# ArjunNarayanan/ProximalPolicyOptimization.jl

Hardware: AMD Instinct MI355X
Metric: env-steps/sec end-to-end PPO (rollout+GAE+update), 4096 envs, 1/2/4/8 MI355X (higher is better)
Workload: dtype f32; 1 GPU; 4096 parallel synthetic rand-poly-shaped envs per GPU (Q=8,H=32,A=128,F=72 int8), 2x256 MLP policy fp32, T=128 steps/iteration, 4 epochs, minibatch 4096/GPU, gamma=1.0 eps=0.05 entropy_w=0.01 Adam 1e-4; returns mode (lambda=1,V=0); envs_per_gpu=4096, T=128, epochs=4, minibatch_per_gpu=4096, parallelism=dp1, rollouts_streamed_to_disk=False

## Files before the change

### proximalpolicyoptimization.jl_amd/csrc/ppo_optim.hip

```cpp
#include "ppo_internal.h"
#include "ppo_device.h"
#include <algorithm>
#include <cstring>
#include <type_traits>

struct ParamLayout {
    int F, HID, NT, FP, NI, NL2;
    int64_t offW1, offb1, offW2, offW3, offb3, np;
};

static ParamLayout layout_of(const ppo_policy_s* p) {
    ParamLayout L;
    L.F = p->F; L.HID = p->HID; L.NT = p->HID / 32; L.FP = ((p->F + 31) / 32) * 32; L.NI = L.FP / 32; L.NL2 = p->L - 1;
    L.offW1 = 0; L.offb1 = (int64_t)p->HID * p->F; L.offW2 = L.offb1 + p->HID;
    L.offW3 = L.offW2 + (int64_t)L.NL2 * ((int64_t)p->HID * p->HID + p->HID);
    L.offb3 = L.offW3 + (int64_t)PPO_OUT * p->HID; L.np = L.offb3 + PPO_OUT;
    return L;
}

__device__ void loss_reduce_block(const double* __restrict__ terms, int64_t B, double inv_Bg, double entropy_weight,
                                  float* __restrict__ grad_tail);

struct PackPtrs {
    float* w1p; float* w2p; float* w2tp; float* b1p; float* b2p; float* w3p; float* b3;
    uint16_t* w1b; uint16_t* w2b; uint16_t* w2tb; uint16_t* w3c; uint16_t* w3tb;
    uint16_t* w2x; uint16_t* w1x; uint16_t* w2fx;
};

struct AdamFuse { float* params; float* m; float* v; double eta, beta1, beta2, eps, bp1, bp2; float* hist2; int on; };
__device__ __forceinline__ void pack_one(const ParamLayout& L, const PackPtrs& P, int64_t i, float x);
__device__ __forceinline__ void adam_one(const AdamFuse& A, const ParamLayout& L, const PackPtrs& P, int64_t i, float g);

struct ChainFuse {
    float* params; float* hist2; int on; int n;
    int kind[4];
    double c[4][6];
    float* s0[4]; float* s1[4];
};
__device__ __forceinline__ void chain_one(const ChainFuse& C, const ParamLayout& L, const PackPtrs& P, int64_t i, float g);
__device__ __forceinline__ void fuse_one(const AdamFuse& A, const ParamLayout& L, const PackPtrs& P, int64_t i, float g) { adam_one(A, L, P, i, g); }
__device__ __forceinline__ void fuse_one(const ChainFuse& C, const ParamLayout& L, const PackPtrs& P, int64_t i, float g) { chain_one(C, L, P, i, g); }

struct ClipFuse {
    float* hist2; int on;
    ChainFuse C;
    float* dbuf;
    double* part;
};
__device__ __forceinline__ float chain_delta(const ChainFuse& C, int64_t i, float g);
__device__ __forceinline__ void clip_partial(double* __restrict__ part, size_t e, float d);

__device__ __forceinline__ void fuse_one(const ClipFuse&, const ParamLayout&, const PackPtrs&, int64_t, float) {}

template <typename Fuse>
__global__ __launch_bounds__(256) void k_grad_reduce(const float* __restrict__ slabs, size_t slab_stride, int nwg_w, int nwg_s, ParamLayout L,
                                                     float* __restrict__ grad, const double* __restrict__ terms, int64_t B,
                                                     double inv_Bg, double entropy_weight, Fuse A, PackPtrs P) {
    if (blockIdx.x == gridDim.x - 1) {
        loss_reduce_block(terms, B, inv_Bg, entropy_weight, grad + L.np);
        if (A.on && A.hist2 && threadIdx.x == 0) { A.hist2[0] = grad[L.np]; A.hist2[1] = grad[L.np + 1]; }
        return;
    }
    __shared__ float part[4][64];
    const int el = threadIdx.x & 63, grp = threadIdx.x >> 6;
    const size_t e = (size_t)blockIdx.x * 64 + el;
    const size_t nW2l = (size_t)L.HID * L.HID, nW2 = (size_t)L.NL2 * nW2l, nW1 = (size_t)L.HID * L.FP;
    const size_t total = nW2 + nW1 + (size_t)L.HID * (1 + L.NL2) + (size_t)L.HID * 4 + 4;
    float ps[8] = {0.f, 0.f, 0.f, 0.f, 0.f, 0.f, 0.f, 0.f};
    const int nwg = (e < nW2 + nW1) ? nwg_w : nwg_s;
    bool dead = false;
    if (e >= nW2 && e < nW2 + nW1) {
        const size_t e1 = e - nW2;
        const int it = (int)((e1 >> 10) % L.NI);
        dead = 32 * it + (int)(e1 & 31) >= L.F;
    }
    if (e < total && !dead) {
        int g = grp;
        for (; g + 28 < nwg; g += 32) {
#pragma unroll
            for (int u = 0; u < 8; ++u) ps[u] += slabs[(size_t)(g + 4 * u) * slab_stride + e];
        }
        for (int u = 0; g < nwg; g += 4, ++u) ps[u] += slabs[(size_t)g * slab_stride + e];
    }
    part[grp][el] = ((ps[0] + ps[1]) + (ps[2] + ps[3])) + ((ps[4] + ps[5]) + (ps[6] + ps[7]));
    __syncthreads();
    constexpr bool clip = std::is_same<Fuse, ClipFuse>::value;
    if (grp != 0 || (e >= total && !clip)) return;
    const float s = (part[0][el] + part[1][el]) + (part[2][el] + part[3][el]);
    int64_t canon = -1;
    if (e < nW2) {
        const int lay = (int)(e / nW2l);
        const size_t el2 = e - (size_t)lay * nW2l;
        const int lane = (int)(el2 & 63), r = (int)((el2 >> 6) & 15);
        const int tile = (int)(el2 >> 10), kt = tile % L.NT, ft = tile / L.NT;
        const int f = dfeat(ft, r, lane >> 5), k = 32 * kt + (lane & 31);
        canon = L.offW2 + (int64_t)lay * ((int64_t)nW2l + L.HID) + f + (int64_t)L.HID * k;
    } else if (e < nW2 + nW1) {
        const size_t e1 = e - nW2;
        const int lane = (int)(e1 & 63), r = (int)((e1 >> 6) & 15);
        const int tile = (int)(e1 >> 10), it = tile % L.NI, ft = tile / L.NI;
        const int ko = dfeat(ft, r, lane >> 5), i = 32 * it + (lane & 31);
        if (i < L.F) canon = L.offW1 + ko + (int64_t)L.HID * i;
    } else {
        size_t e2 = e - nW2 - nW1;
        if (e2 < (size_t)L.HID) canon = L.offb1 + (int64_t)e2;
        else if ((e2 -= L.HID) < (size_t)L.HID * L.NL2)
            canon = L.offW2 + (int64_t)(e2 / L.HID) * ((int64_t)nW2l + L.HID) + (int64_t)nW2l + (int64_t)(e2 % L.HID);
        else if ((e2 -= (size_t)L.HID * L.NL2) < (size_t)L.HID * 4) canon = L.offW3 + (int64_t)(e2 & 3) + 4 * (int64_t)(e2 >> 2);
        else canon = L.offb3 + (int64_t)(e2 - (size_t)L.HID * 4);
    }
    if constexpr (clip) {
        float d = 0.f;
        if (e < total && canon >= 0) {
            grad[canon] = s;
            d = chain_delta(A.C, canon, s);
            A.dbuf[canon] = d;
        }
        clip_partial(A.part, e, d);
        return;
    }
    if (canon >= 0) {
        grad[canon] = s;
        if (A.on) fuse_one(A, L, P, canon, s);
    }
}

__device__ void loss_reduce_block(const double* __restrict__ terms, int64_t B, double inv_Bg, double entropy_weight,
                                  float* __restrict__ grad_tail) {
    __shared__ double s0[256], s1[256];
    const double2* t2 = reinterpret_cast<const double2*>(terms);
    double a[8] = {0, 0, 0, 0, 0, 0, 0, 0}, b[8] = {0, 0, 0, 0, 0, 0, 0, 0};
    int64_t i = threadIdx.x;
    for (; i + 7 * 256 < B; i += 8 * 256) {
#pragma unroll
        for (int u = 0; u < 8; ++u) { const double2 v = t2[i + u * 256]; a[u] += v.x; b[u] += v.y; }
    }
    for (int u = 0; i < B; i += 256, ++u) { const double2 v = t2[i]; a[u] += v.x; b[u] += v.y; }
    s0[threadIdx.x] = ((a[0] + a[1]) + (a[2] + a[3])) + ((a[4] + a[5]) + (a[6] + a[7]));
    s1[threadIdx.x] = ((b[0] + b[1]) + (b[2] + b[3])) + ((b[4] + b[5]) + (b[6] + b[7]));
    __syncthreads();
    for (int off = 128; off >= 1; off >>= 1) {
        if ((int)threadIdx.x < off) { s0[threadIdx.x] += s0[threadIdx.x + off]; s1[threadIdx.x] += s1[threadIdx.x + off]; }
        __syncthreads();
    }
    if (threadIdx.x == 0) {
        grad_tail[0] = (float)(-(s0[0] * inv_Bg));
        grad_tail[1] = (float)(entropy_weight * (-(s1[0] * inv_Bg)));
    }
}


__device__ __forceinline__ uint16_t to_bf16(float x) { return __builtin_bit_cast(uint16_t, (__bf16)x); }
__device__ __forceinline__ void split3_bf16(float x, uint16_t& ph, uint16_t& pm, uint16_t& pl) {
    ph = to_bf16(x);
    const float r1 = x - __uint_as_float((uint32_t)ph << 16);
    pm = to_bf16(r1);
    const float r2 = r1 - __uint_as_float((uint32_t)pm << 16);
    pl = to_bf16(r2);
}
__device__ __forceinline__ void acc_kslot(int kk, int& s, int& hh, int& jj) {
    const int q = kk & 15;
    s = kk >> 4; hh = (q >> 2) & 1; jj = 4 * (q >> 3) + (q & 3);
}

__device__ __forceinline__ void pack_one(const ParamLayout& L, const PackPtrs& P, int64_t i, float x) {
    const int HID = L.HID, F = L.F, NT = L.NT;
    if (i < L.offb1) {
        const int io = (int)(i % HID), k = (int)(i / HID);
        const int hh = k / (F / 2), s = k % (F / 2);
        P.w1p[((size_t)((io >> 5) * (F / 8) + (s >> 2)) * 64 + (io & 31) + 32 * hh) * 4 + (s & 3)] = x;
        if (P.w1x) {
            uint16_t ph, pm, pl;
            split3_bf16(x, ph, pm, pl);
            uint16_t* base = P.w1x + ((size_t)(io >> 5) * 5 + (k >> 4)) * 3 * 512 + ((size_t)(io & 31) + 32 * ((k >> 3) & 1)) * 8 + (k & 7);
            base[0] = pl; base[512] = pm; base[1024] = ph;
        }
        if (P.w1b) {
            const int KS1 = (F + 15) / 16;
            P.w1b[((size_t)((io >> 5) * KS1 + (k >> 4)) * 64 + (io & 31) + 32 * ((k >> 3) & 1)) * 8 + (k & 7)] = to_bf16(x);
        }
    } else if (i < L.offW2) {
        const int f = (int)(i - L.offb1), kk = f & 31, hh = (kk >> 2) & 1, r = (kk & 3) + 4 * (kk >> 3);
        P.b1p[((f >> 5) * 2 + hh) * 16 + r] = x;
    } else if (i < L.offW3) {
        const int64_t per = (int64_t)HID * HID + HID;
        const int lay = (int)((i - L.offW2) / per);
        const int64_t e = (i - L.offW2) - (int64_t)lay * per;
        if (e >= (int64_t)HID * HID) {
            const int f = (int)(e - (int64_t)HID * HID), kk = f & 31, hh = (kk >> 2) & 1, r = (kk & 3) + 4 * (kk >> 3);
            P.b2p[(size_t)lay * HID + ((f >> 5) * 2 + hh) * 16 + r] = x;
            return;
        }
        const size_t lo = (size_t)lay * HID * HID;
        const int f = (int)(e % HID), k = (int)(e / HID);
        {
            const int kk = k & 31, hh = (kk >> 2) & 1, r = (kk & 3) + 4 * (kk >> 3);
            const int s = 16 * (k >> 5) + r;
            P.w2p[lo + ((size_t)((f >> 5) * (HID / 8) + (s >> 2)) * 64 + (f & 31) + 32 * hh) * 4 + (s & 3)] = x;
        }
        {
            const bool zrow = PPO_BWD_Z2ROW_AT(HID);
            const int g = f >> 3, hh = zrow ? (f >> 2) & 1 : f & 1, e = zrow ? f & 3 : (f >> 1) & 3;
            P.w2tp[lo + ((size_t)((k >> 5) * (HID / 8) + g) * 64 + (k & 31) + 32 * hh) * 4 + e] = x;
        }
        if (P.w2x && lay == 0) {
            uint16_t ph, pm, pl;
            split3_bf16(x, ph, pm, pl);
            const int KS = HID / 16;
            int s, hh, jj;
            {
                acc_kslot(f & 31, s, hh, jj);
                uint16_t* base = P.w2x + ((size_t)(k >> 5) * KS + 2 * (f >> 5) + s) * 3 * 512 + ((size_t)(k & 31) + 32 * hh) * 8 + jj;
                base[0] = pl; base[512] = pm; base[1024] = ph;
            }
            {
                acc_kslot(k & 31, s, hh, jj);
                uint16_t* base = P.w2fx + ((size_t)(f >> 5) * KS + 2 * (k >> 5) + s) * 3 * 512 + ((size_t)(f & 31) + 32 * hh) * 8 + jj;
                base[0] = pl; base[512] = pm; base[1024] = ph;
            }
        }
        if (P.w2b) {
            const uint16_t xb = to_bf16(x);
            int s, hh, jj;
            acc_kslot(k & 31, s, hh, jj);
            P.w2b[((size_t)((f >> 5) * (HID / 16) + 2 * (k >> 5) + s) * 64 + (f & 31) + 32 * hh) * 8 + jj] = xb;
            P.w2tb[((size_t)((k >> 5) * (HID / 16) + (f >> 4)) * 64 + (k & 31) + 32 * ((f >> 3) & 1)) * 8 + (f & 7)] = xb;
        }
    } else if (i < L.offb3) {
        const int64_t e = i - L.offW3;
        const int oo = (int)(e & 3), k = (int)(e >> 2);
        const int kk = k & 31, hh = (kk >> 2) & 1, r = (kk & 3) + 4 * (kk >> 3);
        P.w3p[((size_t)(hh * NT + (k >> 5)) * 16 + r) * 4 + oo] = x;
        if (P.w3c) {
            const uint16_t xb = to_bf16(x);
            int s, h2, jj;
            acc_kslot(k & 31, s, h2, jj);
            P.w3c[((size_t)((2 * (k >> 5) + s) * 2 + h2) * 4 + oo) * 8 + jj] = xb;
            P.w3tb[(size_t)k * 4 + oo] = xb;
        }
    } else {
        P.b3[i - L.offb3] = x;
    }
}

__device__ __forceinline__ void adam_one(const AdamFuse& A, const ParamLayout& L, const PackPtrs& P, int64_t i, float g) {
    const double gd = (double)g;
    const float mn = (float)(A.beta1 * (double)A.m[i] + (1.0 - A.beta1) * gd);
    const float vn = (float)(A.beta2 * (double)A.v[i] + ((1.0 - A.beta2) * gd) * gd);
    A.m[i] = mn; A.v[i] = vn;
    const double delta = (double)mn / (1.0 - A.bp1) / (sqrt((double)vn / (1.0 - A.bp2)) + A.eps) * A.eta;
    const float x = A.params[i] - (float)delta;
    A.params[i] = x;
    pack_one(L, P, i, x);
}

__global__ void k_pack_params(const float* __restrict__ params, ParamLayout L, PackPtrs P) {
    const int64_t i = (int64_t)blockIdx.x * blockDim.x + threadIdx.x;
    if (i >= L.np) return;
    pack_one(L, P, i, params[i]);
}

__global__ void k_adam(float* __restrict__ params, const float* __restrict__ grad, float* __restrict__ m,
                       float* __restrict__ v, ParamLayout L, PackPtrs P, double eta, double beta1, double beta2,
                       double eps, double bp1, double bp2, float* __restrict__ hist2) {
    const int64_t i = (int64_t)blockIdx.x * blockDim.x + threadIdx.x;
    if (hist2 && i < 2) hist2[i] = grad[L.np + i];
    if (i >= L.np) return;
    const double gd = (double)grad[i];
    const float mn = (float)(beta1 * (double)m[i] + (1.0 - beta1) * gd);
    const float vn = (float)(beta2 * (double)v[i] + ((1.0 - beta2) * gd) * gd);
    m[i] = mn; v[i] = vn;
    const double delta = (double)mn / (1.0 - bp1) / (sqrt((double)vn / (1.0 - bp2)) + eps) * eta;
    const float x = params[i] - (float)delta;
    params[i] = x;
    pack_one(L, P, i, x);
}

__device__ __forceinline__ float chain_delta(const ChainFuse& C, int64_t i, float g) {
    float d = g;
#pragma unroll
    for (int j = 0; j < 4; ++j) {
        if (j >= C.n) break;
        const double* c = C.c[j];
        const double dd = (double)d;
        const int kind = C.kind[j];
        if (kind == PPO_OPT_ADAM) {
            float* m = C.s0[j];
            float* v = C.s1[j];
            const float mn = (float)(c[1] * (double)m[i] + (1.0 - c[1]) * dd);
            const float vn = (float)(c[2] * (double)v[i] + ((1.0 - c[2]) * dd) * dd);
            m[i] = mn; v[i] = vn;
            d = (float)((double)mn / (1.0 - c[4]) / (sqrt((double)vn / (1.0 - c[5])) + c[3]) * c[0]);
        } else if (kind == PPO_OPT_EXPDECAY || kind == PPO_OPT_DESCENT) {
            d = (float)(dd * c[0]);
        } else if (kind == PPO_OPT_MOMENTUM) {
            const float vn = (float)(c[1] * (double)C.s0[j][i] - c[0] * dd);
            C.s0[j][i] = vn;
            d = -vn;
        } else if (kind == PPO_OPT_NESTEROV) {
            const double v0 = (double)C.s0[j][i];
            const double dn = (c[1] * c[1]) * v0 - ((1.0 + c[1]) * c[0]) * dd;
            C.s0[j][i] = (float)(c[1] * v0 - c[0] * dd);
            d = (float)(-dn);
        } else if (kind == PPO_OPT_RMSPROP) {
            const float a = (float)(c[1] * (double)C.s0[j][i] + ((1.0 - c[1]) * dd) * dd);
            C.s0[j][i] = a;
            const float ra = (float)sqrt((double)a);
            d = (float)(dd * (c[0] / ((double)ra + c[2])));
        } else if (kind == PPO_OPT_CLIPVALUE) {
            d = (float)(dd > c[0] ? c[0] : (dd < -c[0] ? -c[0] : dd));
        } else if (kind == PPO_OPT_WEIGHTDECAY) {
            d = (float)(dd + c[0] * (double)C.params[i]);
        } else {
            d = (float)(dd * c[0]);
        }
    }
    return d;
}

__device__ __forceinline__ void dd_add(double& h, double& l, double bh, double bl) {
    const double s = h + bh;
    if (!isfinite(s)) { h = s; l = 0.0; return; }
    const double v = s - h;
    double e = (h - (s - v)) + (bh - v);
    e += l + bl;
    h = s + e;
    l = e - (h - s);
}

__device__ __forceinline__ void clip_partial(double* __restrict__ part, size_t e, float d) {
    double h = (double)d * (double)d, l = 0.0;
#pragma unroll
    for (int off = 16; off >= 1; off >>= 1) {
        const double bh = __shfl_down(h, off, 32), bl = __shfl_down(l, off, 32);
        dd_add(h, l, bh, bl);
    }
    if ((e & 31) == 0) { part[2 * (e >> 5)] = h; part[2 * (e >> 5) + 1] = l; }
}

__device__ __forceinline__ void chain_one(const ChainFuse& C, const ParamLayout& L, const PackPtrs& P, int64_t i, float g) {
    const float x = C.params[i] - chain_delta(C, i, g);
    C.params[i] = x;
    pack_one(L, P, i, x);
}

__global__ void k_chain_update(const float* __restrict__ grad, ParamLayout L, PackPtrs P, ChainFuse C) {
    const int64_t i = (int64_t)blockIdx.x * blockDim.x + threadIdx.x;
    if (C.hist2 && i < 2) C.hist2[i] = grad[L.np + i];
    if (i >= L.np) return;
    chain_one(C, L, P, i, grad[i]);
}

__global__ __launch_bounds__(256) void k_chain_clip1(const float* __restrict__ grad, ParamLayout L, ClipFuse A) {
    const int64_t i = (int64_t)blockIdx.x * blockDim.x + threadIdx.x;
    if (A.hist2 && i < 2) A.hist2[i] = grad[L.np + i];
    float d = 0.f;
    if (i < L.np) {
        d = chain_delta(A.C, i, grad[i]);
        A.dbuf[i] = d;
    }
    clip_partial(A.part, (size_t)i, d);
}

#define PPO_CLIP_MAX_ARRAYS 10
struct ClipMap {
    const float* dbuf; const double* part;
    double thresh;
    int na;
    int64_t start[PPO_CLIP_MAX_ARRAYS + 1];
    int32_t s0[PPO_CLIP_MAX_ARRAYS], s1[PPO_CLIP_MAX_ARRAYS];
};
__device__ __forceinline__ int clip_array(const ClipMap& M, int64_t i) {
    int a = 0;
    while (a + 1 < M.na && i >= M.start[a + 1]) ++a;
    return a;
}

#define PPO_CLIP_BLOCK 256
__global__ __launch_bounds__(PPO_CLIP_BLOCK) void k_clip_apply(ParamLayout L, PackPtrs P, ChainFuse C, ClipMap M) {
    __shared__ double wsum[PPO_CLIP_BLOCK / 64][2];
    __shared__ float nrm[PPO_CLIP_MAX_ARRAYS];
    const int t = threadIdx.x, lane = t & 63, w = t >> 6;
    const int64_t i0 = (int64_t)blockIdx.x * PPO_CLIP_BLOCK, i = i0 + t;
    const int a0 = clip_array(M, i0), a1 = clip_array(M, std::min<int64_t>(i0 + PPO_CLIP_BLOCK, L.np) - 1);
// ... 279 lines not shown
```

### proximalpolicyoptimization.jl_amd/csrc/ppo_policy_bwd_x6.hip

```cpp
#include "ppo_internal.h"
#include "ppo_device.h"
#include <cstdlib>

#include "ppo_x6.h"
typedef float pk2 __attribute__((ext_vector_type(2)));
__device__ __forceinline__ pk2 pk_fma(pk2 a, pk2 b, pk2 c) { return __builtin_elementwise_fma(a, b, c); }

struct BwdXArgs {
    unsigned long long* stamps;
    const int8_t* states; const int32_t* idx; int64_t B;
    int tps; int x_by_tile;
    const float4* act1; const float4* act2; const float4* dY;
    const uint4* w2x; const float4* w3p;
    float* slabs; size_t slab_stride;
};

template <int F, int HID>
struct XCfg {
    static_assert(F == 72, "state rows of 72 features (+ the ones column, zero padded to 96)");
    static constexpr int NT = HID / 32, KS = HID / 16;
    static constexpr int LD = 36;
    static constexpr int WG_PER_CU = HID == 128 ? 2 : 1;
    static constexpr int XROW = 80;
    static constexpr int NIX = 3;
    static constexpr size_t oZ2 = 0, szZ2 = (size_t)NT * 6 * 1024;
    static constexpr size_t oH2 = oZ2 + szZ2, szH2 = sizeof(float) * HID * LD;
    static constexpr size_t oH1 = oH2 + szH2, szH1 = (size_t)3 * NT * 2048;
    static constexpr size_t oX = oH1 + szH1, szX = (size_t)32 * NIX * XROW;
    static constexpr size_t oDY = oX + szX, oW3 = oDY + 512, oID = oW3 + (size_t)HID * 16, total = oID + 2048;
    static_assert(total <= 160 * 1024 / WG_PER_CU, "LDS budget");
};

#define X6_LANE() unsigned ln = (unsigned)lane; asm volatile("" : "+v"(ln)); const int j = (int)(ln & 31u), h = (int)(ln >> 5); (void)j; (void)h

#ifndef PPO_X6_DMA_SPREAD
#define PPO_X6_DMA_SPREAD 0
#endif
#ifndef PPO_X6_RING
#define PPO_X6_RING 6
#endif
#ifndef PPO_X6_RING_256
#define PPO_X6_RING_256 4
#endif

template <int F, int HID>
__global__ __launch_bounds__(HID * 2, 2) void k_policy_bwd_x6(BwdXArgs a) {
    using C = XCfg<F, HID>;
    constexpr int NT = C::NT, KS = C::KS, NTHR = NT * 64, LD = C::LD, NIX = C::NIX, XROW = C::XROW;
    constexpr int XQW = 32 * F / 8, XPD = (XQW + NTHR - 1) / NTHR;
    constexpr int RD = HID >= 256 ? PPO_X6_RING_256 : PPO_X6_RING;
    static_assert(NTHR >= 256 && NTHR >= HID, "shape");
    extern __shared__ __attribute__((aligned(16))) char smem_c[];
    char* const fragZ2 = smem_c + C::oZ2;
    float* const sH2 = reinterpret_cast<float*>(smem_c + C::oH2);
    char* const imgH1 = smem_c + C::oH1;
    char* const imgX = smem_c + C::oX;
    float* const sDY = reinterpret_cast<float*>(smem_c + C::oDY);
    float* const sW3 = reinterpret_cast<float*>(smem_c + C::oW3);
    uint4* const sID = reinterpret_cast<uint4*>(smem_c + C::oID);

    const int tid = threadIdx.x, lane = tid & 63;
    const int w = __builtin_amdgcn_readfirstlane(tid >> 6);
    const int j = lane & 31, h = lane >> 5;

    f32x16 accW2[NT], accW1[NIX];
#pragma unroll
    for (int kt = 0; kt < NT; ++kt)
#pragma unroll
        for (int r = 0; r < 16; ++r) accW2[kt][r] = 0.0f;
#pragma unroll
    for (int it = 0; it < NIX; ++it)
#pragma unroll
        for (int r = 0; r < 16; ++r) accW1[it][r] = 0.0f;
    float db2 = 0.f, db3 = 0.f, dw3[4] = {0.f, 0.f, 0.f, 0.f};

#ifdef PPO_X6_ZERO_LDS
    for (int i = tid; i < (int)(C::total / 4); i += NTHR) reinterpret_cast<uint32_t*>(smem_c)[i] = 0u;
    __syncthreads();
#endif
    if (tid < HID) {
        const int kk = tid & 31, hh = (kk >> 2) & 1, r = (kk & 3) + 4 * (kk >> 3);
        *reinterpret_cast<float4*>(&sW3[tid * 4]) = a.w3p[(size_t)(hh * NT + (tid >> 5)) * 16 + r];
    }
    if (tid < 64) {
        const int n = tid & 31, hB = tid >> 5, e = 4 * ((n >> 3) & 1) + (n & 3);
#pragma unroll
        for (int s1 = 0; s1 < 2; ++s1) {
            uint4 v = make_uint4(0u, 0u, 0u, 0u);
            if (hB == ((n >> 2) & 1) && s1 == (n >> 4)) {
                const uint32_t one = (e & 1) ? 0x3F800000u : 0x00003F80u;
                if ((e >> 1) == 0) v.x = one; else if ((e >> 1) == 1) v.y = one; else if ((e >> 1) == 2) v.z = one; else v.w = one;
            }
            sID[s1 * 64 + tid] = v;
        }
    }
    for (int i = tid; i < 32 * NIX * XROW / 4; i += NTHR) {
        const int row = i / (XROW / 4), c = i % (XROW / 4);
        reinterpret_cast<uint32_t*>(imgX)[i] = (row == F && c < 16) ? 0x3F803F80u : 0u;
    }
    __syncthreads();

    const char* const wx = reinterpret_cast<const char*>(a.w2x + (size_t)w * 3 * KS * 64);
    float* const h2slice = sH2 + (size_t)(32 * w) * LD;
    char* const z2own = fragZ2 + (size_t)w * 6 * 1024;
    const unsigned h2slice_lds = __builtin_amdgcn_readfirstlane((unsigned)(size_t)(__attribute__((address_space(3))) void*)h2slice);
    const unsigned z2own_lds = __builtin_amdgcn_readfirstlane((unsigned)(size_t)(__attribute__((address_space(3))) void*)z2own);
    auto dma_frag = [&](const float4* base, int64_t t, unsigned dst_lds, unsigned ln) {
        const float4* const sb = base + ((size_t)t * NT + w) * 4 * 64;
        const unsigned voff = ln * 16u;
#pragma unroll
        for (int q = 0; q < 4; ++q) {
            unsigned keep;
            const float4* gsrc = sb + q * 64;
            const unsigned dst = dst_lds + (unsigned)q * 1024u;
            asm volatile("s_mov_b32 %0, m0\n\ts_mov_b32 m0, %2\n\ts_nop 0\n\tglobal_load_lds_dwordx4 %1, %3 nt\n\ts_mov_b32 m0, %0"
                         : "=&s"(keep) : "v"(voff), "s"(dst), "s"(gsrc) : "memory");
        }
    };
    auto dma_one = [&](const float4* base, int64_t t, unsigned dst_lds, int q, unsigned ln) {
        unsigned keep;
        const float4* gsrc = base + ((size_t)t * NT + w) * 4 * 64 + ln + q * 64;
        const unsigned dst = dst_lds + (unsigned)q * 1024u;
        asm volatile("s_mov_b32 %0, m0\n\ts_mov_b32 m0, %2\n\ts_nop 0\n\tglobal_load_lds_dwordx4 %1, off nt\n\ts_mov_b32 m0, %0"
                     : "=&s"(keep) : "v"(gsrc), "s"(dst) : "memory");
    };
    (void)dma_one;
    float4 dy;
    uint2 xd[XPD];
    auto issue_tile_loads = [&](int64_t t, int sidx, unsigned ln) {
        dy = *reinterpret_cast<const float4*>(reinterpret_cast<const char*>(a.dY + (size_t)t * 32) + (ln & 31u) * 16u);
        const char* xs = reinterpret_cast<const char*>(a.states + (a.x_by_tile ? (size_t)t : ((size_t)sidx * a.tps + (size_t)(t % a.tps))) * 32 * F);
#pragma unroll
        for (int i = 0; i < XPD; ++i) {
            const unsigned u = (unsigned)(64 * w) + ln + (unsigned)i * NTHR;
            const unsigned d = (u & 31u) * (unsigned)(F / 8) + (u >> 5);
            xd[i] = u < (unsigned)XQW ? *reinterpret_cast<const uint2*>(xs + d * 8u) : make_uint2(0u, 0u);
        }
    };
    if ((int64_t)blockIdx.x < a.B) {
        dma_frag(a.act2, blockIdx.x, h2slice_lds, (unsigned)lane);
        dma_frag(a.act1, blockIdx.x, z2own_lds, (unsigned)lane);
        issue_tile_loads(blockIdx.x, a.x_by_tile ? 0 : __builtin_amdgcn_readfirstlane(a.idx[blockIdx.x / a.tps]), (unsigned)lane);
    }
    asm volatile("s_waitcnt vmcnt(0)" ::: "memory");
    __syncthreads();

#ifdef PPO_X6_STAMP
    unsigned long long st_sum[12] = {0, 0, 0, 0, 0, 0, 0, 0, 0, 0, 0, 0}, st_t = clock64();
#define XSTAMP(i) do { unsigned long long _n = clock64(); st_sum[i] += _n - st_t; st_t = _n; } while (0)
#else
#define XSTAMP(i) do {} while (0)
#endif
    for (int64_t tile = blockIdx.x; tile < a.B; tile += gridDim.x) {
        {
            X6_LANE();
            const unsigned hw = (unsigned)(w * 2048 + 64 * j), cx = (unsigned)(j >> 2) & 7u;
            float4 v1[4];
#pragma unroll
            for (int q = 0; q < 4; ++q) v1[q] = *reinterpret_cast<const float4*>(z2own + q * 1024 + ln * 16);
            asm volatile("s_waitcnt lgkmcnt(0)" ::: "memory");
#pragma unroll
            for (int q = 0; q < 4; ++q) {
                const float hv[4] = {v1[q].x, v1[q].y, v1[q].z, v1[q].w};
                uint2 ph, pm, pl;
                x_split4(hv, ph, pm, pl);
                const unsigned off = hw + 8u * (((unsigned)(2 * q + h)) ^ cx);
                *reinterpret_cast<uint2*>(imgH1 + off) = ph;
                *reinterpret_cast<uint2*>(imgH1 + NT * 2048 + off) = pm;
                *reinterpret_cast<uint2*>(imgH1 + 2 * NT * 2048 + off) = pl;
            }
        }
        __builtin_amdgcn_sched_barrier(0);
        XSTAMP(0);
        {
            X6_LANE();
            float* const h2b = sH2 + (32 * w + 4 * h) * LD + j;
            const float w3a0 = sW3[(32 * w + j) * 4 + h], w3a1 = sW3[(32 * w + j) * 4 + 2 + h];
            float4 v2[4];
#pragma unroll
            for (int q = 0; q < 4; ++q) v2[q] = *reinterpret_cast<const float4*>(h2slice + q * 256 + ln * 4);
            if (w == 0 && h == 0) *reinterpret_cast<float4*>(&sDY[j * 4]) = dy;
            f32x16 dh2;
#pragma unroll
            for (int r = 0; r < 16; ++r) dh2[r] = 0.0f;
            dh2 = __builtin_amdgcn_mfma_f32_32x32x2f32(w3a0, h ? dy.y : dy.x, dh2, 0, 0, 0);
            dh2 = __builtin_amdgcn_mfma_f32_32x32x2f32(w3a1, h ? dy.w : dy.z, dh2, 0, 0, 0);
            asm volatile("s_waitcnt lgkmcnt(0)" ::: "memory");
#pragma unroll
            for (int s = 0; s < 2; ++s) {
                uint2 zh[2], zm[2], zl[2];
#pragma unroll
                for (int qq = 0; qq < 2; ++qq) {
                    const int q = 2 * s + qq;
                    const float h2v[4] = {v2[q].x, v2[q].y, v2[q].z, v2[q].w};
                    float z[4];
#pragma unroll
                    for (int e = 0; e < 4; ++e) {
                        z[e] = dh2[4 * q + e] * (h2v[e] > 0.0f ? 1.0f : 0.01f);
                        h2b[(e + 8 * q) * LD] = h2v[e];
                    }
                    x_split4(z, zh[qq], zm[qq], zl[qq]);
                }
                *reinterpret_cast<uint4*>(z2own + (s * 3 + 0) * 1024 + ln * 16) = make_uint4(zh[0].x, zh[0].y, zh[1].x, zh[1].y);
                *reinterpret_cast<uint4*>(z2own + (s * 3 + 1) * 1024 + ln * 16) = make_uint4(zm[0].x, zm[0].y, zm[1].x, zm[1].y);
                *reinterpret_cast<uint4*>(z2own + (s * 3 + 2) * 1024 + ln * 16) = make_uint4(zl[0].x, zl[0].y, zl[1].x, zl[1].y);
                __builtin_amdgcn_sched_barrier(0);
            }
        }
        XSTAMP(1);
        {
        X6_LANE();
#pragma unroll
        for (int i = 0; i < XPD; ++i) {
            const int d = 64 * w + (int)ln + i * NTHR;
            if (d < XQW) {
                const int row = d & 31, c = d >> 5;
                const int slot = (row & 19) | ((row & 4) << 1) | ((row & 8) >> 1);
                const uint32_t xw[2] = {xd[i].x, xd[i].y};
                char* const xp = imgX + (8 * c) * XROW + 2 * slot;
#pragma unroll
                for (int e = 0; e < 8; ++e) {
                    const float xv = (float)(int)(int8_t)(xw[e >> 2] >> (8 * (e & 3)));
                    *reinterpret_cast<uint16_t*>(xp + e * XROW) = (uint16_t)(__float_as_uint(xv) >> 16);
                }
            }
        }
        }
        XSTAMP(2);
        __syncthreads();
        XSTAMP(3);
        auto small_grads = [&]() {
            X6_LANE();
            const float* gh = sH2 + (32 * w + j) * LD + 16 * h;
            const float* gy = sDY + 64 * h;
            pk2 d01 = {0.f, 0.f}, d23 = {0.f, 0.f};
#pragma unroll 1
            for (int rc = 0; rc < 16; rc += 4) {
                const float4 h4 = *reinterpret_cast<const float4*>(gh + rc);
                const float hv[4] = {h4.x, h4.y, h4.z, h4.w};
                float4 y[4];
#pragma unroll
                for (int i = 0; i < 4; ++i) y[i] = *reinterpret_cast<const float4*>(gy + (rc + i) * 4);
                __builtin_amdgcn_sched_barrier(0);
#pragma unroll
                for (int i = 0; i < 4; ++i) {
                    const pk2 hh2 = {hv[i], hv[i]};
                    d01 = pk_fma(pk2{y[i].x, y[i].y}, hh2, d01); d23 = pk_fma(pk2{y[i].z, y[i].w}, hh2, d23);
                }
                __builtin_amdgcn_sched_barrier(0);
            }
            dw3[0] += d01.x; dw3[1] += d01.y; dw3[2] += d23.x; dw3[3] += d23.y;
            if (w == 0 && ln < 4u) {
                float s = 0.f;
                for (int r = 0; r < 32; ++r) s += sDY[r * 4 + ln];
                db3 += s;
            }
        };
        uint4 ring[RD];
#pragma unroll
        for (int g = 0; g < RD; ++g) { unsigned lo = (unsigned)lane * 16u; asm volatile("" : "+v"(lo)); ring[g] = *reinterpret_cast<const uint4*>(wx + (lo + (unsigned)g * 1024u)); }
        const bool grads_first = (2 * w < NT);
        const int64_t ntile = (tile + gridDim.x < a.B) ? tile + gridDim.x : tile;
        if (grads_first) small_grads();
        XSTAMP(4);
        {
            f32x16 acc;
#pragma unroll
            for (int r = 0; r < 16; ++r) acc[r] = 0.0f;
            f32x16 accs;
#pragma unroll
            for (int r = 0; r < 16; ++r) accs[r] = 0.0f;
            unsigned wo = (unsigned)RD * 1024u;
            asm volatile("" : "+s"(wo));
            constexpr int RU = (RD % 3 == 0) ? RD / 3 : RD;
            static_assert(KS % RU == 0 && (3 * RU) % RD == 0, "ring rounds");
            static_assert(RD * 1024 <= PPO_X6_W2_PAD_BYTES, "the last ring round reads RD pieces past the end of the W2 stream");
            unsigned zo = (unsigned)lane * 16u;
            asm volatile("" : "+v"(zo));
            const char* zp = fragZ2 + zo;
            const unsigned lo16 = zo;
#pragma unroll 1
            for (int k0 = 0; k0 < KS; k0 += RU) {
#pragma unroll
                for (int u = 0; u < RU; ++u) {
                    const int s0 = (3 * u + 0) % RD, s1 = (3 * u + 1) % RD, s2 = (3 * u + 2) % RD;
                    const uint4 z_h = *reinterpret_cast<const uint4*>(zp + (u * 3 + 0) * 1024);
                    const uint4 z_m = *reinterpret_cast<const uint4*>(zp + (u * 3 + 1) * 1024);
                    const uint4 z_l = *reinterpret_cast<const uint4*>(zp + (u * 3 + 2) * 1024);
                    accs = x_mfma(z_h, ring[s0], accs);
                    __builtin_amdgcn_sched_barrier(0);
                    ring[s0] = *reinterpret_cast<const uint4*>(wx + (lo16 + wo));
                    __builtin_amdgcn_sched_barrier(0);
                    accs = x_mfma(z_m, ring[s1], accs);
                    accs = x_mfma(z_h, ring[s1], accs);
                    __builtin_amdgcn_sched_barrier(0);
                    ring[s1] = *reinterpret_cast<const uint4*>(wx + (lo16 + wo + 1024u));
                    __builtin_amdgcn_sched_barrier(0);
                    accs = x_mfma(z_l, ring[s2], accs);
                    accs = x_mfma(z_m, ring[s2], accs);
                    acc = x_mfma(z_h, ring[s2], acc);
                    __builtin_amdgcn_sched_barrier(0);
                    ring[s2] = *reinterpret_cast<const uint4*>(wx + (lo16 + wo + 2048u));
                    wo += 3 * 1024;
                    asm volatile("" : "+s"(wo));
                    __builtin_amdgcn_sched_barrier(0);
                }
                zp += RU * 3 * 1024;
            }
#pragma unroll
            for (int r = 0; r < 16; ++r) acc[r] = acc[r] + accs[r];
            XSTAMP(5);
            X6_LANE();
            const unsigned q4 = (ln & 15u) >> 2, p4 = ln & 3u, g1 = (ln >> 4) & 1u;
            typedef __attribute__((address_space(3))) xs16x4 lds_s16x4;
            uint2 zh[4], zm[4], zl[4];
#pragma unroll
            for (int g = 0; g < 4; ++g) {
                const unsigned r0 = 8u * g + 4u * h;
                const char* hp = imgH1 + w * 2048 + 64u * (r0 + q4) + 8u * ((4u * g1 + p4) ^ ((r0 >> 2) & 7u));
                const uint2 sg = __builtin_bit_cast(uint2, __builtin_amdgcn_ds_read_tr16_b64_v4i16((lds_s16x4*)(hp)));
                const float z1[4] = {acc[4 * g + 0] * ((int16_t)(sg.x & 0xFFFFu) > 0 ? 1.0f : 0.01f),
                                     acc[4 * g + 1] * ((int32_t)sg.x >= 0x10000 ? 1.0f : 0.01f),
                                     acc[4 * g + 2] * ((int16_t)(sg.y & 0xFFFFu) > 0 ? 1.0f : 0.01f),
                                     acc[4 * g + 3] * ((int32_t)sg.y >= 0x10000 ? 1.0f : 0.01f)};
                x_split4(z1, zh[g], zm[g], zl[g]);
            }
            const char* const xb = imgX + j * XROW + 16 * h;
#pragma unroll
            for (int s = 0; s < 2; ++s) {
                uint4 bx[NIX];
#pragma unroll
                for (int it = 0; it < NIX; ++it) bx[it] = *reinterpret_cast<const uint4*>(xb + 32 * it * XROW + 32 * s);
                const uint4 a_l = make_uint4(zl[2 * s].x, zl[2 * s].y, zl[2 * s + 1].x, zl[2 * s + 1].y);
                const uint4 a_m = make_uint4(zm[2 * s].x, zm[2 * s].y, zm[2 * s + 1].x, zm[2 * s + 1].y);
                const uint4 a_h = make_uint4(zh[2 * s].x, zh[2 * s].y, zh[2 * s + 1].x, zh[2 * s + 1].y);
#pragma unroll
                for (int it = 0; it < NIX; ++it) {
                    accW1[it] = x_mfma(a_l, bx[it], accW1[it]);
                    accW1[it] = x_mfma(a_m, bx[it], accW1[it]);
                    accW1[it] = x_mfma(a_h, bx[it], accW1[it]);
                }
            }
        }
        XSTAMP(6);
        if (!grads_first) small_grads();
        XSTAMP(7);
        __syncthreads();
        XSTAMP(8);
        {
            X6_LANE();
            uint4 ah[2], am[2], al[2];
            {
                const uint4 id0 = sID[ln], id1 = sID[64 + ln];
                float s2 = 0.f;
#pragma unroll
                for (int p = 2; p >= 0; --p) {
                    const uint4 f0 = *reinterpret_cast<const uint4*>(z2own + (0 * 3 + p) * 1024 + ln * 16);
                    const uint4 f1 = *reinterpret_cast<const uint4*>(z2own + (1 * 3 + p) * 1024 + ln * 16);
                    f32x16 t;
#pragma unroll
                    for (int r = 0; r < 16; ++r) t[r] = 0.0f;
                    t = x_mfma(f0, id0, t);
                    t = x_mfma(f1, id1, t);
                    float sp = 0.f;
#pragma unroll
                    for (int r = 0; r < 16; ++r) sp += t[r];
                    s2 += sp;
                    uint4 pk[2];
#pragma unroll
                    for (int s = 0; s < 2; ++s)
                        pk[s] = make_uint4(x_perm(t[8 * s + 0], t[8 * s + 1]), x_perm(t[8 * s + 2], t[8 * s + 3]),
                                           x_perm(t[8 * s + 4], t[8 * s + 5]), x_perm(t[8 * s + 6], t[8 * s + 7]));
                    if (p == 0) { ah[0] = pk[0]; ah[1] = pk[1]; } else if (p == 1) { am[0] = pk[0]; am[1] = pk[1]; } else { al[0] = pk[0]; al[1] = pk[1]; }
                }
                db2 += s2;
            }
            asm volatile("s_waitcnt lgkmcnt(0)" ::: "memory");
#if !(PPO_X6_DMA_SPREAD & 1)
            dma_frag(a.act2, ntile, h2slice_lds, ln);
#endif
#if !(PPO_X6_DMA_SPREAD & 2)
            dma_frag(a.act1, ntile, z2own_lds, ln);
#endif
            {
                int nidx = 0;
                if (!a.x_by_tile) {
                    const int32_t* ip = a.idx + ntile / a.tps;
                    asm volatile("s_load_dword %0, %1, 0x0\n\ts_waitcnt lgkmcnt(0)" : "=s"(nidx) : "s"(ip) : "memory");
                }
                issue_tile_loads(ntile, nidx, ln);
            }
            unsigned tb[2][2];
            {
                const unsigned q4 = (ln & 15u) >> 2, p4 = ln & 3u, g1 = (ln >> 4) & 1u;
#pragma unroll
                for (int s = 0; s < 2; ++s)
#pragma unroll
                    for (int u = 0; u < 2; ++u) {
                        const unsigned r0 = 16u * s + 8u * u + 4u * h;
                        tb[s][u] = 64u * (r0 + q4) + 8u * ((4u * g1 + p4) ^ ((r0 >> 2) & 7u));
                    }
                asm volatile("" : "+v"(tb[0][0]), "+v"(tb[0][1]), "+v"(tb[1][0]), "+v"(tb[1][1]));
            }
            auto load_b = [&](int g, uint4 (&b)[3]) {
                const char* i0 = imgH1 + (g >> 1) * 2048;
                const int s = g & 1;
                b[0] = x_tr_frag(i0 + tb[s][0], i0 + tb[s][1]);
                b[1] = x_tr_frag(i0 + NT * 2048 + tb[s][0], i0 + NT * 2048 + tb[s][1]);
                b[2] = x_tr_frag(i0 + 2 * NT * 2048 + tb[s][0], i0 + 2 * NT * 2048 + tb[s][1]);
            };
            XSTAMP(9);
            uint4 bc[3], bn[3];
            load_b(0, bc);
#pragma unroll
            for (int g = 0; g < 2 * NT; ++g) {
                const int kt = g >> 1, s = g & 1;
                if (g + 1 < 2 * NT) load_b(g + 1, bn);
                __builtin_amdgcn_sched_barrier(0);
                accW2[kt] = x_mfma(al[s], bc[0], accW2[kt]);
                accW2[kt] = x_mfma(am[s], bc[1], accW2[kt]);
                accW2[kt] = x_mfma(ah[s], bc[2], accW2[kt]);
                accW2[kt] = x_mfma(am[s], bc[0], accW2[kt]);
                accW2[kt] = x_mfma(ah[s], bc[1], accW2[kt]);
                accW2[kt] = x_mfma(ah[s], bc[0], accW2[kt]);
                __builtin_amdgcn_sched_barrier(0);
#if PPO_X6_DMA_SPREAD
                if ((PPO_X6_DMA_SPREAD & 1) && g < 4) dma_one(a.act2, ntile, h2slice_lds, g, ln);
                else if ((PPO_X6_DMA_SPREAD & 2) && g >= 4 && g < 8) dma_one(a.act1, ntile, z2own_lds, g - 4, ln);
                __builtin_amdgcn_sched_barrier(0);
#endif
#pragma unroll
                for (int p = 0; p < 3; ++p) bc[p] = bn[p];
            }
        }
        XSTAMP(10);
        asm volatile("s_waitcnt vmcnt(0)" ::: "memory");
        __syncthreads();
        XSTAMP(11);
    }
#ifdef PPO_X6_STAMP
    if (a.stamps && lane == 0 && (w == 0 || w == NT - 1))
        for (int i = 0; i < 12; ++i) a.stamps[((size_t)blockIdx.x * 2 + (w ? 1 : 0)) * 12 + i] = st_sum[i];
#endif

    constexpr int FP = 96, NI = FP / 32;
    float* slab = a.slabs + (size_t)blockIdx.x * a.slab_stride;
    float* sW2 = slab;
    float* sW1 = sW2 + (size_t)HID * HID;
    float* sb1 = sW1 + (size_t)HID * FP;
    float* sb2 = sb1 + HID;
    float* sw3 = sb2 + HID;
    float* sb3 = sw3 + HID * 4;
    unsigned l4 = (unsigned)lane * 4u;
    asm volatile("" : "+v"(l4));
#pragma unroll
    for (int kt = 0; kt < NT; ++kt) {
        const uint64_t tb = x_uniform_addr(sW2 + (size_t)(w * NT + kt) * 16 * 64);
#pragma unroll
        for (int r = 0; r < 16; ++r) *x_gptr<float>(tb, l4 + (unsigned)r * 256u) = accW2[kt][r];
    }
#pragma unroll
    for (int it = 0; it < NI; ++it) {
        if (32 * it + j >= F) continue;
        const uint64_t tb = x_uniform_addr(sW1 + (size_t)(w * NI + it) * 16 * 64);
#pragma unroll
        for (int r = 0; r < 16; ++r) *x_gptr<float>(tb, l4 + (unsigned)r * 256u) = accW1[it][r];
    }
    if (j == F - 64) {
#pragma unroll
        for (int r = 0; r < 16; ++r) sb1[32 * w + (r & 3) + 8 * (r >> 2) + 4 * h] = accW1[2][r];
    }
    {
        db2 += __shfl_xor(db2, 32);
#pragma unroll
        for (int i = 0; i < 4; ++i) dw3[i] += __shfl_xor(dw3[i], 32);
        if (h == 0) {
            const int f = 32 * w + j;
            sb2[f] = db2;
            *reinterpret_cast<float4*>(&sw3[f * 4]) = make_float4(dw3[0], dw3[1], dw3[2], dw3[3]);
        }
    }
    if (tid < 4) sb3[tid] = db3;
    asm volatile("s_waitcnt vmcnt(0)" ::: "memory");
}

#ifdef PPO_X6_STAMP
static unsigned long long* g_x6_stamps = nullptr;
extern "C" int32_t ppo_debug_x6_stamps(unsigned long long* out) {
    if (!g_x6_stamps) return -1;
    (void)hipDeviceSynchronize();
    return hipMemcpy(out, g_x6_stamps, 512 * 24 * 8, hipMemcpyDeviceToHost) == hipSuccess ? 0 : -2;
}
#endif

int32_t launch_policy_bwd_x6(ppo_policy_s* p, ppo_rollouts_s* ro, const int32_t* idx_dev, int64_t B) {
    BwdXArgs a;
    a.stamps = nullptr;
#ifdef PPO_X6_STAMP
    { if (!g_x6_stamps) (void)hipMalloc((void**)&g_x6_stamps, 512 * 24 * 8); a.stamps = g_x6_stamps; }
#endif
    a.tps = ro->H / 32;
    a.states = ro->compact ? p->xs.p : ro->states.p; a.x_by_tile = ro->compact ? 1 : 0;
    a.idx = idx_dev; a.B = B * a.tps;
    a.act1 = (const float4*)p->act1.p; a.act2 = (const float4*)p->act2.p; a.dY = (const float4*)p->dY.p;
    a.w2x = (const uint4*)p->w2x.p; a.w3p = (const float4*)p->w3p.p;
    a.slabs = p->slabs.p; a.slab_stride = slab_floats(p->F, p->HID);
    int nwg = 0;
    ProfScope ps("k_policy_bwd");
#define LAUNCH(FF, HH)                                                                                        \
    do {                                                                                                      \
        const int64_t cap = 256 * XCfg<FF, HH>::WG_PER_CU;                                                    \
        nwg = (int)(a.B < cap ? a.B : cap);                                                                   \
        p->nwg_bwd = nwg; p->nwg_small = 0;                                                                   \
        const size_t lds = XCfg<FF, HH>::total;                                                               \
        static thread_local bool attr_set = false;                                                            \
        if (!attr_set) {                                                                                      \
            HIP_TRY(hipFuncSetAttribute((const void*)k_policy_bwd_x6<FF, HH>,                                 \
                                        hipFuncAttributeMaxDynamicSharedMemorySize, (int)lds));               \
            attr_set = true;                                                                                  \
        }                                                                                                     \
        hipLaunchKernelGGL((k_policy_bwd_x6<FF, HH>), dim3(nwg), dim3(HH * 2), lds, ppo_stream(), a);          \
    } while (0)
    if (p->HID == 256) LAUNCH(72, 256);
    else LAUNCH(72, 128);
#undef LAUNCH
    HIP_TRY(hipGetLastError());
    return PPO_OK;
}
```

Baseline: 2.481 million env-steps/s.

## Overlap bwd prologue and slab stores with tile loop; software-pipeline slab reduction loads

The backward kernel now issues the first tile's DMA before its shared-memory setup (W3, identity fragments, X image), so that setup runs while the loads are in flight and one barrier is dropped. The loop body becomes a lambda with a compile-time 'last' flag. The final iteration skips the next-tile prefetch and trailing sync and writes the W1 and W2 gradient slabs interleaved with its last MFMAs. The next-tile index scalar load is issued earlier so its latency hides behind other work. The optimizer's slab reduction double-buffers 8-wide loads to keep more memory requests outstanding, at the cost of more code and register pressure.

```diff
diff --git a/proximalpolicyoptimization.jl_amd/csrc/ppo_optim.hip b/proximalpolicyoptimization.jl_amd/csrc/ppo_optim.hip
--- a/proximalpolicyoptimization.jl_amd/csrc/ppo_optim.hip
+++ b/proximalpolicyoptimization.jl_amd/csrc/ppo_optim.hip
@@ -75,11 +75,24 @@
         dead = 32 * it + (int)(e1 & 31) >= L.F;
     }
     if (e < total && !dead) {
-        int g = grp;
-        for (; g + 28 < nwg; g += 32) {
-#pragma unroll
-            for (int u = 0; u < 8; ++u) ps[u] += slabs[(size_t)(g + 4 * u) * slab_stride + e];
-        }
+        const int R = grp + 28 < nwg ? (nwg - 29 - grp) / 32 + 1 : 0;
+        const float* const col = slabs + (size_t)grp * slab_stride + e;
+        const size_t rs = 32 * slab_stride, us = 4 * slab_stride;
+        float va[8], vb[8];
+#define LOAD8(v, r) _Pragma("unroll") for (int u = 0; u < 8; ++u) v[u] = col[(size_t)(r) * rs + (size_t)u * us]
+#define ADD8(v) _Pragma("unroll") for (int u = 0; u < 8; ++u) ps[u] += v[u]
+        if (R == 1) { LOAD8(va, 0); ADD8(va); }
+        else if (R >= 2) {
+            LOAD8(va, 0); LOAD8(vb, 1);
+            int r = 2;
+            for (; r + 2 <= R; r += 2) { ADD8(va); LOAD8(va, r); ADD8(vb); LOAD8(vb, r + 1); }
+            ADD8(va);
+            if (r < R) { LOAD8(va, r); ADD8(vb); ADD8(va); }
+            else ADD8(vb);
+        }
+#undef LOAD8
+#undef ADD8
+        int g = grp + 32 * R;
         for (int u = 0; g < nwg; g += 4, ++u) ps[u] += slabs[(size_t)g * slab_stride + e];
     }
     part[grp][el] = ((ps[0] + ps[1]) + (ps[2] + ps[3])) + ((ps[4] + ps[5]) + (ps[6] + ps[7]));
diff --git a/proximalpolicyoptimization.jl_amd/csrc/ppo_policy_bwd_x6.hip b/proximalpolicyoptimization.jl_amd/csrc/ppo_policy_bwd_x6.hip
--- a/proximalpolicyoptimization.jl_amd/csrc/ppo_policy_bwd_x6.hip
+++ b/proximalpolicyoptimization.jl_amd/csrc/ppo_policy_bwd_x6.hip
@@ -63,6 +63,9 @@
     const int w = __builtin_amdgcn_readfirstlane(tid >> 6);
     const int j = lane & 31, h = lane >> 5;
 
+#ifdef PPO_X6_STAMP
+    const unsigned long long st_t0 = clock64();
+#endif
     f32x16 accW2[NT], accW1[NIX];
 #pragma unroll
     for (int kt = 0; kt < NT; ++kt)
@@ -78,28 +81,6 @@
     for (int i = tid; i < (int)(C::total / 4); i += NTHR) reinterpret_cast<uint32_t*>(smem_c)[i] = 0u;
     __syncthreads();
 #endif
-    if (tid < HID) {
-        const int kk = tid & 31, hh = (kk >> 2) & 1, r = (kk & 3) + 4 * (kk >> 3);
-        *reinterpret_cast<float4*>(&sW3[tid * 4]) = a.w3p[(size_t)(hh * NT + (tid >> 5)) * 16 + r];
-    }
-    if (tid < 64) {
-        const int n = tid & 31, hB = tid >> 5, e = 4 * ((n >> 3) & 1) + (n & 3);
-#pragma unroll
-        for (int s1 = 0; s1 < 2; ++s1) {
-            uint4 v = make_uint4(0u, 0u, 0u, 0u);
-            if (hB == ((n >> 2) & 1) && s1 == (n >> 4)) {
-                const uint32_t one = (e & 1) ? 0x3F800000u : 0x00003F80u;
-                if ((e >> 1) == 0) v.x = one; else if ((e >> 1) == 1) v.y = one; else if ((e >> 1) == 2) v.z = one; else v.w = one;
-            }
-            sID[s1 * 64 + tid] = v;
-        }
-    }
-    for (int i = tid; i < 32 * NIX * XROW / 4; i += NTHR) {
-        const int row = i / (XROW / 4), c = i % (XROW / 4);
-        reinterpret_cast<uint32_t*>(imgX)[i] = (row == F && c < 16) ? 0x3F803F80u : 0u;
-    }
-    __syncthreads();
-
     const char* const wx = reinterpret_cast<const char*>(a.w2x + (size_t)w * 3 * KS * 64);
     float* const h2slice = sH2 + (size_t)(32 * w) * LD;
     char* const z2own = fragZ2 + (size_t)w * 6 * 1024;
@@ -142,16 +123,62 @@
         dma_frag(a.act1, blockIdx.x, z2own_lds, (unsigned)lane);
         issue_tile_loads(blockIdx.x, a.x_by_tile ? 0 : __builtin_amdgcn_readfirstlane(a.idx[blockIdx.x / a.tps]), (unsigned)lane);
     }
+    if (tid < HID) {
+        const int kk = tid & 31, hh = (kk >> 2) & 1, r = (kk & 3) + 4 * (kk >> 3);
+        *reinterpret_cast<float4*>(&sW3[tid * 4]) = a.w3p[(size_t)(hh * NT + (tid >> 5)) * 16 + r];
+    }
+    if (tid < 64) {
+        const int n = tid & 31, hB = tid >> 5, e = 4 * ((n >> 3) & 1) + (n & 3);
+#pragma unroll
+        for (int s1 = 0; s1 < 2; ++s1) {
+            uint4 v = make_uint4(0u, 0u, 0u, 0u);
+            if (hB == ((n >> 2) & 1) && s1 == (n >> 4)) {
+                const uint32_t one = (e & 1) ? 0x3F800000u : 0x00003F80u;
+                if ((e >> 1) == 0) v.x = one; else if ((e >> 1) == 1) v.y = one; else if ((e >> 1) == 2) v.z = one; else v.w = one;
+            }
+            sID[s1 * 64 + tid] = v;
+        }
+    }
+    for (int i = tid; i < 32 * NIX * XROW / 4; i += NTHR) {
+        const int row = i / (XROW / 4), c = i % (XROW / 4);
+        reinterpret_cast<uint32_t*>(imgX)[i] = (row == F && c < 16) ? 0x3F803F80u : 0u;
+    }
     asm volatile("s_waitcnt vmcnt(0)" ::: "memory");
     __syncthreads();
 
 #ifdef PPO_X6_STAMP
-    unsigned long long st_sum[12] = {0, 0, 0, 0, 0, 0, 0, 0, 0, 0, 0, 0}, st_t = clock64();
+    unsigned long long st_sum[14] = {0, 0, 0, 0, 0, 0, 0, 0, 0, 0, 0, 0, 0, 0}, st_t = clock64();
+    st_sum[12] = st_t - st_t0;
 #define XSTAMP(i) do { unsigned long long _n = clock64(); st_sum[i] += _n - st_t; st_t = _n; } while (0)
 #else
 #define XSTAMP(i) do {} while (0)
 #endif
-    for (int64_t tile = blockIdx.x; tile < a.B; tile += gridDim.x) {
+    constexpr int FP = 96, NI = FP / 32;
+    static_assert(NI == NIX, "input tiles");
+    auto slab_ptr = [&]() { return a.slabs + (size_t)blockIdx.x * a.slab_stride; };
+    auto store_w2 = [&](int kt, int r0, int r1, unsigned ln) {
+        const uint64_t tb = x_uniform_addr(slab_ptr() + (size_t)(w * NT + kt) * 16 * 64);
+#pragma unroll
+        for (int r = r0; r < r1; ++r) *x_gptr<float>(tb, ln * 4u + (unsigned)r * 256u) = accW2[kt][r];
+    };
+    auto store_w1 = [&](unsigned ln) {
+        const int jj = (int)(ln & 31u), hh = (int)(ln >> 5);
+        float* const sW1 = slab_ptr() + (size_t)HID * HID;
+#pragma unroll
+        for (int it = 0; it < NI; ++it) {
+            if (32 * it + jj >= F) continue;
+            const uint64_t tb = x_uniform_addr(sW1 + (size_t)(w * NI + it) * 16 * 64);
+#pragma unroll
+            for (int r = 0; r < 16; ++r) *x_gptr<float>(tb, ln * 4u + (unsigned)r * 256u) = accW1[it][r];
+        }
+        if (jj == F - 64) {
+            float* const sb1 = sW1 + (size_t)HID * FP;
+#pragma unroll
+            for (int r = 0; r < 16; ++r) sb1[32 * w + (r & 3) + 8 * (r >> 2) + 4 * hh] = accW1[2][r];
+        }
+    };
+    auto body = [&](const int64_t tile, auto last_c) {
+        constexpr bool Last = decltype(last_c)::value;
         {
             X6_LANE();
             const unsigned hw = (unsigned)(w * 2048 + 64 * j), cx = (unsigned)(j >> 2) & 7u;
@@ -260,7 +287,7 @@
 #pragma unroll
         for (int g = 0; g < RD; ++g) { unsigned lo = (unsigned)lane * 16u; asm volatile("" : "+v"(lo)); ring[g] = *reinterpret_cast<const uint4*>(wx + (lo + (unsigned)g * 1024u)); }
         const bool grads_first = (2 * w < NT);
-        const int64_t ntile = (tile + gridDim.x < a.B) ? tile + gridDim.x : tile;
+        const int64_t ntile = tile + gridDim.x;
         if (grads_first) small_grads();
         XSTAMP(4);
         {
@@ -342,6 +369,7 @@
                 }
             }
         }
+        if constexpr (Last) { X6_LANE(); store_w1(ln); }
         XSTAMP(6);
         if (!grads_first) small_grads();
         XSTAMP(7);
@@ -349,6 +377,13 @@
         XSTAMP(8);
         {
             X6_LANE();
+            int nidx = 0;
+            if constexpr (!Last) {
+                if (!a.x_by_tile) {
+                    const int32_t* ip = a.idx + ntile / a.tps;
+                    asm volatile("s_load_dword %0, %1, 0x0" : "=s"(nidx) : "s"(ip) : "memory");
+                }
+            }
             uint4 ah[2], am[2], al[2];
             {
                 const uint4 id0 = sID[ln], id1 = sID[64 + ln];
@@ -376,18 +411,14 @@
                 db2 += s2;
             }
             asm volatile("s_waitcnt lgkmcnt(0)" ::: "memory");
+            if constexpr (!Last) {
 #if !(PPO_X6_DMA_SPREAD & 1)
             dma_frag(a.act2, ntile, h2slice_lds, ln);
 #endif
 #if !(PPO_X6_DMA_SPREAD & 2)
             dma_frag(a.act1, ntile, z2own_lds, ln);
 #endif
-            {
-                int nidx = 0;
-                if (!a.x_by_tile) {
-                    const int32_t* ip = a.idx + ntile / a.tps;
-                    asm volatile("s_load_dword %0, %1, 0x0\n\ts_waitcnt lgkmcnt(0)" : "=s"(nidx) : "s"(ip) : "memory");
-                }
+                asm volatile("s_waitcnt lgkmcnt(0)" : "+s"(nidx) :: "memory");
                 issue_tile_loads(ntile, nidx, ln);
             }
             unsigned tb[2][2];
@@ -424,8 +455,11 @@
                 accW2[kt] = x_mfma(ah[s], bc[1], accW2[kt]);
                 accW2[kt] = x_mfma(ah[s], bc[0], accW2[kt]);
                 __builtin_amdgcn_sched_barrier(0);
+                if constexpr (Last) {
+                    if (kt > 0) { store_w2(kt - 1, 8 * s, 8 * s + 8, ln); __builtin_amdgcn_sched_barrier(0); }
+                }
 #if PPO_X6_DMA_SPREAD
-                if ((PPO_X6_DMA_SPREAD & 1) && g < 4) dma_one(a.act2, ntile, h2slice_lds, g, ln);
+                if (Last) {} else if ((PPO_X6_DMA_SPREAD & 1) && g < 4) dma_one(a.act2, ntile, h2slice_lds, g, ln);
                 else if ((PPO_X6_DMA_SPREAD & 2) && g >= 4 && g < 8) dma_one(a.act1, ntile, z2own_lds, g - 4, ln);
                 __builtin_amdgcn_sched_barrier(0);
 #endif
@@ -434,41 +468,27 @@
             }
         }
         XSTAMP(10);
+        if constexpr (!Last) {
         asm volatile("s_waitcnt vmcnt(0)" ::: "memory");
         __syncthreads();
+        }
         XSTAMP(11);
-    }
-#ifdef PPO_X6_STAMP
-    if (a.stamps && lane == 0 && (w == 0 || w == NT - 1))
-        for (int i = 0; i < 12; ++i) a.stamps[((size_t)blockIdx.x * 2 + (w ? 1 : 0)) * 12 + i] = st_sum[i];
-#endif
-
-    constexpr int FP = 96, NI = FP / 32;
-    float* slab = a.slabs + (size_t)blockIdx.x * a.slab_stride;
-    float* sW2 = slab;
-    float* sW1 = sW2 + (size_t)HID * HID;
-    float* sb1 = sW1 + (size_t)HID * FP;
-    float* sb2 = sb1 + HID;
-    float* sw3 = sb2 + HID;
-    float* sb3 = sw3 + HID * 4;
-    unsigned l4 = (unsigned)lane * 4u;
-    asm volatile("" : "+v"(l4));
-#pragma unroll
-    for (int kt = 0; kt < NT; ++kt) {
-        const uint64_t tb = x_uniform_addr(sW2 + (size_t)(w * NT + kt) * 16 * 64);
-#pragma unroll
-        for (int r = 0; r < 16; ++r) *x_gptr<float>(tb, l4 + (unsigned)r * 256u) = accW2[kt][r];
-    }
-#pragma unroll
-    for (int it = 0; it < NI; ++it) {
-        if (32 * it + j >= F) continue;
-        const uint64_t tb = x_uniform_addr(sW1 + (size_t)(w * NI + it) * 16 * 64);
-#pragma unroll
-        for (int r = 0; r < 16; ++r) *x_gptr<float>(tb, l4 + (unsigned)r * 256u) = accW1[it][r];
-    }
-    if (j == F - 64) {
-#pragma unroll
-        for (int r = 0; r < 16; ++r) sb1[32 * w + (r & 3) + 8 * (r >> 2) + 4 * h] = accW1[2][r];
+    };
+    int64_t tile = blockIdx.x;
+    for (; tile + gridDim.x < a.B; tile += gridDim.x) body(tile, std::false_type{});
+    const bool has_tile = tile < a.B;
+    if (has_tile) body(tile, std::true_type{});
+    float* const sb2 = slab_ptr() + (size_t)HID * HID + (size_t)HID * FP + HID;
+    float* const sw3 = sb2 + HID;
+    float* const sb3 = sw3 + HID * 4;
+    {
+        X6_LANE();
+        if (has_tile) store_w2(NT - 1, 0, 16, ln);
+        else {
+#pragma unroll
+            for (int kt = 0; kt < NT; ++kt) store_w2(kt, 0, 16, ln);
+            store_w1(ln);
+        }
     }
     {
         db2 += __shfl_xor(db2, 32);
@@ -482,6 +502,11 @@
     }
     if (tid < 4) sb3[tid] = db3;
     asm volatile("s_waitcnt vmcnt(0)" ::: "memory");
+#ifdef PPO_X6_STAMP
+    XSTAMP(13);
+    if (a.stamps && lane == 0 && (w == 0 || w == NT - 1))
+        for (int i = 0; i < 14; ++i) a.stamps[((size_t)blockIdx.x * 2 + (w ? 1 : 0)) * 14 + i] = st_sum[i];
+#endif
 }
 
 #ifdef PPO_X6_STAMP
@@ -489,7 +514,7 @@
 extern "C" int32_t ppo_debug_x6_stamps(unsigned long long* out) {
     if (!g_x6_stamps) return -1;
     (void)hipDeviceSynchronize();
-    return hipMemcpy(out, g_x6_stamps, 512 * 24 * 8, hipMemcpyDeviceToHost) == hipSuccess ? 0 : -2;
+    return hipMemcpy(out, g_x6_stamps, 512 * 28 * 8, hipMemcpyDeviceToHost) == hipSuccess ? 0 : -2;
 }
 #endif
 
@@ -497,7 +522,7 @@
     BwdXArgs a;
     a.stamps = nullptr;
 #ifdef PPO_X6_STAMP
-    { if (!g_x6_stamps) (void)hipMalloc((void**)&g_x6_stamps, 512 * 24 * 8); a.stamps = g_x6_stamps; }
+    { if (!g_x6_stamps) (void)hipMalloc((void**)&g_x6_stamps, 512 * 28 * 8); a.stamps = g_x6_stamps; }
 #endif
     a.tps = ro->H / 32;
     a.states = ro->compact ? p->xs.p : ro->states.p; a.x_by_tile = ro->compact ? 1 : 0;
```

Result: no change. 2.505 million env-steps/s, median of 6 (+0.9%).
